# microsoft/AI2BMD

Measured on NVIDIA B200. Metric: MD steps/sec, higher is better.
Workload: dtype f32

## Files before the change

### ai2bmd_b200/csrc/engine.cu

```cuda
#include <cuda_runtime.h>

#include <algorithm>
#include <cmath>
#include <cstdarg>
#include <cstdio>
#include <cstdlib>
#include <cstring>
#include <mutex>
#include <string>
#include <vector>

#include "../../include/visnet_b200.h"
#include "k_edge.cuh"
#include "k_caph.cuh"
#include "k_comm.cuh"
#include "k_edge_tc.cuh"
#include "k_fused.cuh"
#include "k_graph_embed.cuh"
#include <nvtx3/nvToolsExt.h>
#include "k_head.cuh"
#include "k_md.cuh"
#include "k_nonbonded.cuh"
#include "k_restraint.cuh"
#include "k_node.cuh"
// ... 107 lines not shown
    float* d_ef = nullptr;
    int* d_flags = nullptr;
    bool caph_ready = false;
    CaphDev caph{};
    void* caph_mem = nullptr;
    bool comm_ready = false;
    int comm_auto = 1;
    void* comm_base = nullptr;
    void* comm_peer[COMM_MAX_WORLD] = {};
    CommParams comm{};
    int use_graph = 1, npw = 0, te_fwd = 0, te_bwd = 32;
    int use_pdl = 0;
    int npw_opt = 0, te_fwd_opt = 0, edge_tc_opt = -1;
    int tc_rows_opt = 0, tc_rows = 128;
    int tile_rows = 128;
    long long edges_plan = 0;
    int krot = 1;
    int node_nb = 0;
    int node_impl = 1;
    int fused = 0, fused_opt = -1;
    int node_tc = 0, node_tc_opt = -1;
    int embed_batch_opt = -1;
    int edge_tc = -1;
    struct GraphEntry { int kind; StepIO io; cudaGraphExec_t exec; };
    std::vector<GraphEntry> graphs;
    int launches = 0;
    bool accum_dirty = false;
    std::vector<std::string> stage_names;
    bool md_ready = false;
    MdParams md{};
// ... 304 lines not shown
    a.layer = l; a.mw = h->mw; a.ws = h->ws;
    const LayerW& lw = h->mw.layer[l];
    const size_t chunk = 4 * 8192;
    int n = 0;
    a.jobs[n++] = TcJob{lw.tcW1, (int)TC_COL_D0, 0};
    a.jobs[n++] = TcJob{lw.tcW1 + chunk, (int)TC_COL_D1, 0};
    if (l < L - 1) a.jobs[n++] = TcJob{lw.tcW1 + 2 * chunk, (int)TC_COL_D0, 0};
    a.jobs[n++] = TcJob{lw.tcWs, (int)TC_COL_D1, 0};
    a.jobs[n++] = TcJob{lw.tcWs + chunk, (int)TC_COL_D0, 0};
    a.njobs = n;
    a.tl = h->timeline ? h->d_tl + (size_t)l * TC_TL_SLOTS : nullptr;
    a.tile_rows = h->tile_rows;
    const int rows = h->tc_rows;
    const int tiles = (h->ws.Ecap + h->tile_rows - 1) / h->tile_rows;
    const int blocks = std::max(1, std::min(tiles, h->sm_count));
    if (rows == 32) Lc.launch(edge_fwd_tc_kernel<32>, dim3(blocks), dim3(TC2_THREADS), TC_SMEM_BYTES, a);
    else if (rows == 64) Lc.launch(edge_fwd_tc_kernel<64>, dim3(blocks), dim3(TC2_THREADS), TC_SMEM_BYTES, a);
    else if (rows == 96) Lc.launch(edge_fwd_tc_kernel<96>, dim3(blocks), dim3(TC2_THREADS), TC_SMEM_BYTES, a);
    else Lc.launch(edge_fwd_tc_kernel<128>, dim3(blocks), dim3(TC2_THREADS), TC_SMEM_BYTES, a);
    Lc.check();
}

void edge_fwd(Launcher& Lc, int l) {
    if (Lc.h->edge_tc & 1) { launch_edge_fwd_tc(Lc, l); return; }
    if (Lc.h->te_fwd == 64) launch_edge_fwd<64, 8>(Lc, l, 2);
    else launch_edge_fwd<32, 8>(Lc, l, 4);
}
void launch_edge_bwd_tc(Launcher& Lc, int l) {
    vb_handle* h = Lc.h;
    EdgeTcArgs a{};
    a.layer = l; a.mw = h->mw; a.ws = h->ws;
    const LayerW& lw = h->mw.layer[l];
    const size_t chunk = 4 * 8192;
    const bool upd = l < L - 1;
    int n = 0;
    a.jobs[n++] = TcJob{lw.tcWsN, (int)TC_COL_D1, 0};
    a.jobs[n++] = TcJob{lw.tcWsN + chunk, (int)TC_COL_D1, 1};
    a.jobs[n++] = TcJob{lw.tcW1N + chunk, (int)TC_COL_D0, 0};
    a.jobs[n++] = TcJob{lw.tcW1N, (int)TC_COL_D0, 1};
    if (upd) a.jobs[n++] = TcJob{lw.tcW1N + 2 * chunk, (int)TC_COL_D0, 1};
    a.njobs = n;
    a.tl = h->timeline ? h->d_tl + (size_t)(L + l) * TC_TL_SLOTS : nullptr;
    a.tile_rows = h->tile_rows;
    const int rows = h->tc_rows;
    const int tiles = (h->ws.Ecap + h->tile_rows - 1) / h->tile_rows;
    const int blocks = std::max(1, std::min(tiles, h->sm_count));
    if (rows == 32) Lc.launch(edge_bwd_tc_kernel<32>, dim3(blocks), dim3(TC2_THREADS), TC_SMEM_BYTES, a);
    else if (rows == 64) Lc.launch(edge_bwd_tc_kernel<64>, dim3(blocks), dim3(TC2_THREADS), TC_SMEM_BYTES, a);
    else if (rows == 96) Lc.launch(edge_bwd_tc_kernel<96>, dim3(blocks), dim3(TC2_THREADS), TC_SMEM_BYTES, a);
    else Lc.launch(edge_bwd_tc_kernel<128>, dim3(blocks), dim3(TC2_THREADS), TC_SMEM_BYTES, a);
    Lc.check();
}

void edge_bwd(Launcher& Lc, int l) {
    if (Lc.h->edge_tc & 2) { launch_edge_bwd_tc(Lc, l); return; }
    if (Lc.h->te_bwd == 64) launch_edge_bwd<64, 8>(Lc, l, 1);
    else launch_edge_bwd<32, 8>(Lc, l, 2);
}

void fill_fwd_jobs(const LayerW& lw, int l, TcJob* jobs, int& n) {
    const size_t chunk = 4 * 8192;
    n = 0;
    jobs[n++] = TcJob{lw.tcW1, (int)TC_COL_D0, 0};
    jobs[n++] = TcJob{lw.tcW1 + chunk, (int)TC_COL_D1, 0};
    if (l < L - 1) jobs[n++] = TcJob{lw.tcW1 + 2 * chunk, (int)TC_COL_D0, 0};
// ... 210 lines not shown

template <typename K>
cudaError_t opt_in_smem(K kernel, size_t bytes) {
    return cudaFuncSetAttribute(kernel, cudaFuncAttributeMaxDynamicSharedMemorySize, (int)bytes);
}

int configure_kernels(vb_handle* h) {
    CUDA_TRY(h, opt_in_smem(edge_fwd_kernel<32, 8>, edge_fwd_smem_bytes<32>()));
    CUDA_TRY(h, opt_in_smem(edge_fwd_kernel<64, 8>, edge_fwd_smem_bytes<64>()));
    CUDA_TRY(h, opt_in_smem(edge_bwd_kernel<32, 8>, edge_bwd_smem_bytes<32>()));
    CUDA_TRY(h, opt_in_smem(edge_bwd_kernel<64, 8>, edge_bwd_smem_bytes<64>()));
    CUDA_TRY(h, opt_in_smem(node_bwd_kernel<1>, node_bwd_smem_bytes<1>()));
    CUDA_TRY(h, opt_in_smem(node_bwd_kernel<2>, node_bwd_smem_bytes<2>()));
    CUDA_TRY(h, opt_in_smem(head_kernel<1>, HeadSmem<1>::BYTES));
    CUDA_TRY(h, opt_in_smem(head_kernel<2>, HeadSmem<2>::BYTES));
    CUDA_TRY(h, opt_in_smem(edge_fwd_tc_kernel<32>, TC_SMEM_BYTES));
    CUDA_TRY(h, opt_in_smem(edge_fwd_tc_kernel<64>, TC_SMEM_BYTES));
    CUDA_TRY(h, opt_in_smem(edge_fwd_tc_kernel<96>, TC_SMEM_BYTES));
    CUDA_TRY(h, opt_in_smem(edge_fwd_tc_kernel<128>, TC_SMEM_BYTES));
    CUDA_TRY(h, opt_in_smem(edge_bwd_tc_kernel<32>, TC_SMEM_BYTES));
    CUDA_TRY(h, opt_in_smem(edge_bwd_tc_kernel<64>, TC_SMEM_BYTES));
    CUDA_TRY(h, opt_in_smem(edge_bwd_tc_kernel<96>, TC_SMEM_BYTES));
    CUDA_TRY(h, opt_in_smem(edge_bwd_tc_kernel<128>, TC_SMEM_BYTES));
    CUDA_TRY(h, opt_in_smem(fused_fwd_kernel, TC_SMEM_BYTES));
    CUDA_TRY(h, opt_in_smem(fused_bwd_kernel, TC_SMEM_BYTES));
    CUDA_TRY(h, opt_in_smem(node_tc_kernel<NT_OPROJ>, TC_SMEM_BYTES));
    CUDA_TRY(h, opt_in_smem(node_tc_kernel<NT_PROJ>, TC_SMEM_BYTES));
    CUDA_TRY(h, opt_in_smem(node_tc_kernel<NT_BWDA>, TC_SMEM_BYTES));
    CUDA_TRY(h, opt_in_smem(node_tc_kernel<NT_BWDB>, TC_SMEM_BYTES));

    CUDA_TRY(h, opt_in_smem(node_fwd2_kernel<1>, sizeof(NodeFwd2SmemK<1>)));
    CUDA_TRY(h, opt_in_smem(node_bwd2_kernel<1>, sizeof(NodeBwd2SmemK<1>)));
    CUDA_TRY(h, opt_in_smem(node_fwd2_kernel<2>, sizeof(NodeFwd2SmemK<2>)));
    CUDA_TRY(h, opt_in_smem(node_bwd2_kernel<2>, sizeof(NodeBwd2SmemK<2>)));
    CUDA_TRY(h, opt_in_smem(node_fwd2_kernel<3>, sizeof(NodeFwd2SmemK<3>)));
    CUDA_TRY(h, opt_in_smem(node_bwd2_kernel<3>, sizeof(NodeBwd2SmemK<3>)));
    CUDA_TRY(h, opt_in_smem(node_fwd2_kernel<4>, sizeof(NodeFwd2SmemK<4>)));
    CUDA_TRY(h, opt_in_smem(node_bwd2_kernel<4>, sizeof(NodeBwd2SmemK<4>)));
// ... 95 lines not shown
void plan_tiles(vb_handle* h, long long edges) {
    const long long sm = h->sm_count;
    const long long padded = edges + edges * 3 / 100 + 1;
    const long long waves = std::max<long long>(1, (padded + sm * 128 - 1) / (sm * 128));
    long long rpw = (padded + sm * waves * 16 - 1) / (sm * waves * 16);
    if (rpw >= 7) rpw = 8;
    const long long rows = 16 * std::min<long long>(8, std::max<long long>(1, rpw));
    if (h->tc_rows_opt > 0) {
        h->tc_rows = h->tc_rows_opt;
        h->tile_rows = h->tc_rows_opt;
    } else {
        h->tc_rows = rows <= 32 ? 32 : rows <= 64 ? 64 : rows <= 96 ? 96 : 128;
        h->tile_rows = (int)rows;
    }
    h->edges_plan = edges;
}

void choose_defaults(vb_handle* h) {
    const int N = h->ws.N;
    h->npw = h->npw_opt; h->te_fwd = h->te_fwd_opt; h->edge_tc = h->edge_tc_opt;
    h->fused = h->fused_opt >= 0 ? h->fused_opt : 0;
    h->node_tc = h->node_tc_opt >= 0 ? h->node_tc_opt : (N >= 600 ? 1 : 0);
    if (h->fused) h->node_tc = 0;
    set_gxa_parts(h);
    if (h->npw == 0) h->npw = (N > 4096) ? 2 : 1;
    if (h->te_fwd == 0) h->te_fwd = ((long long)N * 17 / 64 >= 2LL * h->sm_count) ? 64 : 32;
    if (h->edge_tc < 0) h->edge_tc = 3;
    plan_tiles(h, h->edges_plan > 0 ? h->edges_plan : (long long)N * 17);
}

// ... 47 lines not shown
    }
    bind_weights(h->mw, h->d_weights);
    h->mw.cutoff = hp->cutoff;
    if (cudaStreamCreateWithFlags(&h->own_stream, cudaStreamNonBlocking) != cudaSuccess) { h->set_error("stream create failed"); return fail(VB_ERR_CUDA); }
    if (configure_kernels(h) != VB_OK) return fail(VB_ERR_CUDA);
    if (const char* s = getenv("VB_USE_GRAPH")) h->use_graph = atoi(s);
    if (const char* s = getenv("VB_NPW")) h->npw_opt = atoi(s);
    if (const char* s = getenv("VB_TE_FWD")) h->te_fwd_opt = atoi(s);
    if (const char* s = getenv("VB_TE_BWD")) h->te_bwd = atoi(s);
    if (const char* s = getenv("VB_EDGE_TC")) h->edge_tc_opt = atoi(s);
    if (const char* s = getenv("VB_USE_PDL")) h->use_pdl = atoi(s) ? 1 : 0;
    if (const char* s = getenv("VB_TC_ROWS")) { const int v = atoi(s); if (v == 32 || v == 64 || v == 96 || v == 128) h->tc_rows_opt = v; }
    if (const char* s = getenv("VB_NODE_IMPL")) h->node_impl = atoi(s);
    if (const char* s = getenv("VB_FUSED")) h->fused_opt = atoi(s) ? 1 : 0;
    if (const char* s = getenv("VB_NODE_TC")) h->node_tc_opt = atoi(s) ? 1 : 0;
    *out = h;
    return VB_OK;
}

void vb_destroy(vb_handle* h) {
    if (!h) return;
    cudaSetDevice(h->device);
    h->drop_graph();
    if (h->own_stream) cudaStreamDestroy(h->own_stream);
    cudaFree(h->d_weights);
    cudaFree(h->d_tl);
    h->free_md();
    h->free_nb();
    h->free_rs();
    h->free_comm();
// ... 695 lines not shown

int vb_set_option(vb_handle* h, const char* key, int64_t value) {
    if (!h || !key) return VB_ERR_ARG;
    std::lock_guard<std::mutex> lk(h->mu);
    const std::string k(key);
    if (k == "use_graph") h->use_graph = (int)value;
    else if (k == "use_pdl" && (value == 0 || value == 1)) h->use_pdl = (int)value;
    else if (k == "npw" && (value == 1 || value == 2)) h->npw = h->npw_opt = (int)value;
    else if (k == "te_fwd" && (value == 32 || value == 64)) h->te_fwd = h->te_fwd_opt = (int)value;
    else if (k == "te_bwd" && (value == 32 || value == 64)) h->te_bwd = (int)value;
    else if (k == "edge_tc" && value >= 0 && value <= 3) h->edge_tc = h->edge_tc_opt = (int)value;
    else if (k == "tc_rows" && (value == 0 || value == 32 || value == 64 || value == 96 || value == 128)) {
        h->tc_rows_opt = (int)value;
        if (h->has_topology) plan_tiles(h, h->edges_plan > 0 ? h->edges_plan : (long long)h->ws.N * 17);
    }
    else if (k == "calibrate" && value == 1) {
        if (!h->has_topology) { h->set_error("vb_set_option: calibrate needs a topology"); return VB_ERR_STATE; }
        int e = 0;
        if (cudaSetDevice(h->device) != cudaSuccess || cudaDeviceSynchronize() != cudaSuccess ||
            cudaMemcpy(&e, h->ws.rowptr + h->ws.N, sizeof(int), cudaMemcpyDeviceToHost) != cudaSuccess) {
            h->set_error("vb_set_option: calibrate failed: %s", cudaGetErrorString(cudaGetLastError()));
            return VB_ERR_CUDA;
        }
        if (e > 0) plan_tiles(h, e);
    }
    else if (k == "node_impl" && (value == 0 || value == 1)) h->node_impl = (int)value;
    else if (k == "node_nb" && (value == 0 || value == 1 || value == 2 || value == 3 || value == 4 || value == 8)) h->node_nb = (int)value;
    else if (k == "krot" && (value == 0 || value == 1)) h->krot = (int)value;
    else if (k == "fused" && (value == 0 || value == 1)) { h->fused = h->fused_opt = (int)value; if (value) h->node_tc = 0; set_gxa_parts(h); }
    else if (k == "node_tc" && (value == 0 || value == 1)) { h->node_tc = h->node_tc_opt = (int)value; if (value) h->fused = 0; set_gxa_parts(h); }
// ... 34 lines not shown
        int v = 0;
        if (!h->caph_ready || cudaDeviceSynchronize() != cudaSuccess ||
            cudaMemcpy(&v, h->caph.evals_out, sizeof(int), cudaMemcpyDeviceToHost) != cudaSuccess) return VB_ERR_STATE;
        return v;
    }
    if (k == "comm_ready") return h->comm_ready ? 1 : 0;
    if (k == "restraints_ready") return h->rs_ready ? 1 : 0;
    if (k == "edge_overflow") {
        int flag = 0;
        if (h->d_flags && cudaMemcpy(&flag, h->d_flags, sizeof(int), cudaMemcpyDeviceToHost) != cudaSuccess) return VB_ERR_CUDA;
        return flag;
    }
    if (k == "timeline") return h->timeline;
    if (k == "tc_rows") return h->tc_rows;
    if (k == "tile_rows") return h->tile_rows;
    if (k == "n_edges_capacity") return h->ws.Ecap;
    return VB_ERR_ARG;
}

int vb_num_stages(const vb_handle* h) { return h ? (int)h->stage_names.size() : 0; }
const char* vb_stage_name(const vb_handle* h, int stage) {
    if (!h || stage < 0 || stage >= (int)h->stage_names.size()) return "";
    return h->stage_names[stage].c_str();
}

int vb_debug_run(vb_handle* h, const float* pos_dev, int n_stages) {
    if (!h) return VB_ERR_ARG;
    std::lock_guard<std::mutex> lk(h->mu);
    if (!h->has_topology || !pos_dev) { h->set_error("vb_debug_run: bad state/arguments"); return VB_ERR_STATE; }
    CUDA_TRY(h, cudaSetDevice(h->device));
// ... 131 lines not shown
```

### ai2bmd_b200/csrc/k_edge_tc.cuh

```cuda
#pragma once
#include "k_edge.cuh"
#include "tc_common.cuh"

namespace vb {

constexpr int TC_TE = 128;
constexpr int TC_STAGES = 4;
constexpr int TC_MAXJOBS = 12;
constexpr int TC_THREADS = 192;
constexpr int TC_LT = D + LDS_PAD;
constexpr int TC_TILE_EXT = 1792;

constexpr uint32_t TC_COL_AHI = 0, TC_COL_ALO = 128, TC_COL_D0 = 256, TC_COL_D1 = 384;

struct TcJob {
    const float* img;
    int d_col;
    int accumulate;
};

struct TcShared {
    alignas(1024) uint8_t ring[TC_STAGES][tc::STAGE_BYTES];
    alignas(16) float tile[TC_TE][TC_LT];
    float tile_ext[TC_TILE_EXT];
// ... 38 lines not shown
    uint32_t phase = 0;
    for (int t = 0; t < ntiles; t++) {
        for (int j = 0; j < njobs; j++) {
            const char* src = reinterpret_cast<const char*>(jobs[j].img);
#pragma unroll 1
            for (int s = 0; s < D / tc::SLAB_K; s++) {
                tc::mbar_wait(&sh.b_empty[stage], phase ^ 1);
                tc::mbar_arrive_expect_tx(&sh.b_full[stage], tc::STAGE_BYTES);
                tc::tma_load_1d(sh.ring[stage], src + (size_t)s * tc::STAGE_BYTES, tc::STAGE_BYTES, &sh.b_full[stage]);
                if (++stage == TC_STAGES) { stage = 0; phase ^= 1; }
            }
        }
    }
}

__device__ __forceinline__ void tc_mma_issuer(TcShared& sh, const TcJob* jobs, int njobs, int ntiles, uint32_t tmem_base,
                                              unsigned long long* tl = nullptr) {
    constexpr uint32_t idesc = tc::idesc_tf32(128, 128);
    int stage = 0;
    uint32_t phase = 0;
    for (int t = 0; t < ntiles; t++) {
        const uint32_t tpar = (uint32_t)(t & 1);
        for (int j = 0; j < njobs; j++) {
            tc::mbar_wait(&sh.go[j], tpar);
            tc::fence_after_sync();
            if (tl != nullptr && t == 0) tl[32 + 2 * j] = (unsigned long long)clock64();
            const uint32_t d_addr = tmem_base + (uint32_t)jobs[j].d_col;
            uint32_t acc = (uint32_t)jobs[j].accumulate;
#pragma unroll 1
            for (int s = 0; s < D / tc::SLAB_K; s++) {
                tc::mbar_wait(&sh.b_full[stage], phase);
                tc::fence_after_sync();
                const uint32_t bhi = tc::smem_u32(sh.ring[stage]);
                const uint32_t blo = bhi + tc::SLAB_BYTES;
#pragma unroll
                for (int kk = 0; kk < tc::SLAB_K / 8; kk++) {
                    const uint32_t a_off = (uint32_t)(s * tc::SLAB_K + kk * 8);
                    const uint64_t dhi = tc::smem_desc_sw128(bhi + kk * 32);
                    const uint64_t dlo = tc::smem_desc_sw128(blo + kk * 32);
                    tc::mma_tf32_ts(d_addr, tmem_base + TC_COL_ALO + a_off, dhi, idesc, acc);
                    tc::mma_tf32_ts(d_addr, tmem_base + TC_COL_AHI + a_off, dlo, idesc, 1u);
                    tc::mma_tf32_ts(d_addr, tmem_base + TC_COL_AHI + a_off, dhi, idesc, 1u);
                    acc = 1u;
                }
                tc::mma_commit(&sh.b_empty[stage]);
                if (++stage == TC_STAGES) { stage = 0; phase ^= 1; }
            }
            tc::mma_commit(&sh.done[j]);
            if (tl != nullptr && t == 0) tl[33 + 2 * j] = (unsigned long long)clock64();
        }
    }
}

__device__ __forceinline__ void tc_signal_go(TcShared& sh, int j) {
    tc::wait_st();
    tc::fence_before_sync();
    tc::mbar_arrive(&sh.go[j]);
// ... 78 lines not shown
        tc::mbar_init(&sh.b_tile, TC2_CWARPS);
        tc::fence_barrier_init();
    }
    if (warp == TC2_CWARPS) tc::tmem_alloc(&sh.tmem_base, 512);
    tc::fence_before_sync();
    __syncthreads();
    tc::fence_after_sync();
    return sh.tmem_base;
}
__device__ __forceinline__ void tc2_teardown(uint32_t tmem_base) {
    tc::fence_before_sync();
    __syncthreads();
    if ((threadIdx.x >> 5) == TC2_CWARPS) tc::tmem_dealloc(tmem_base, 512);
}

template <int ROWS>
__device__ __forceinline__ void tc2_tile_to_a(TcShared& sh, uint32_t tmem, int warp, int lane) {
    if ((warp & 3) * 32 >= ROWS) return;
    const int row = (warp & 3) * 32 + lane, ch = (warp >> 2) * TC2_CBLK;
    const uint32_t tl = tmem + ((uint32_t)((warp & 3) * 32) << 16);
#pragma unroll
    for (int c0 = 0; c0 < TC2_CBLK; c0 += 16) {
        float v[16];
#pragma unroll
        for (int q = 0; q < 16; q += 4) {
            const float4 x = ld4(&sh.tile[row][ch + c0 + q]);
            v[q] = x.x; v[q + 1] = x.y; v[q + 2] = x.z; v[q + 3] = x.w;
        }
        tc::store_a16(tl + TC_COL_AHI, tl + TC_COL_ALO, ch + c0, v);
    }
}
template <int ROWS>
__device__ __forceinline__ void tc2_d_to_tile(TcShared& sh, uint32_t tmem, uint32_t d_col, int warp, int lane) {
    if ((warp & 3) * 32 >= ROWS) return;
    const int row = (warp & 3) * 32 + lane, ch = (warp >> 2) * TC2_CBLK;
    const uint32_t tl = tmem + ((uint32_t)((warp & 3) * 32) << 16) + d_col;
    constexpr int NB16 = TC2_CBLK / 16;
    uint32_t r[NB16][16];
#pragma unroll
    for (int b = 0; b < NB16; b++) tc::tmem_ld16_nowait(tl + ch + b * 16, r[b]);
    tc::wait_ld();
#pragma unroll
    for (int b = 0; b < NB16; b++)
#pragma unroll
        for (int q = 0; q < 16; q += 4)
            st4(&sh.tile[row][ch + b * 16 + q], f4(__uint_as_float(r[b][q]), __uint_as_float(r[b][q + 1]),
                                                    __uint_as_float(r[b][q + 2]), __uint_as_float(r[b][q + 3])));
}
__device__ __forceinline__ void tc2_go(TcShared& sh, int j) {
    tc::wait_st();
    tc::fence_before_sync();
    tc::mbar_arrive(&sh.go[j]);
}

template <int ROWS>
__global__ void __launch_bounds__(TC2_THREADS, 1) edge_fwd_tc_kernel(const __grid_constant__ EdgeTcArgs a) {
    pdl_entry();
    extern __shared__ __align__(1024) uint8_t dyn_raw[];
    TcShared& sh = *tc_shared_base(dyn_raw);
    const Workspace& ws = a.ws;
    const int l = a.layer;
    const LayerW& lw = a.mw.layer[l];
    const bool upd = (l < L - 1);
    const int J_DK = 0, J_DV = 1, J_F = 2, J_S1 = upd ? 3 : 2, J_S2 = upd ? 4 : 3;
    constexpr int RPW = ROWS / TC2_CWARPS;
    const int warp = threadIdx.x >> 5, lane = threadIdx.x & 31, col = lane * 4;
    const int E = ws.rowptr[ws.N];
    const int trows = min(ROWS, max(16, a.tile_rows));
    const int ntiles_total = (E + trows - 1) / trows;
    const int my_tiles = ((int)blockIdx.x < ntiles_total) ? (ntiles_total - (int)blockIdx.x + (int)gridDim.x - 1) / (int)gridDim.x : 0;
    if (a.tl != nullptr && blockIdx.x == 0 && threadIdx.x == 0) a.tl[0] = (unsigned long long)clock64();
    const uint32_t tmem = tc2_setup(sh, a.njobs);
    if (a.tl != nullptr && blockIdx.x == 0 && threadIdx.x == 0) a.tl[1] = (unsigned long long)clock64();

    if (warp == TC2_CWARPS) {
        if (lane == 0) tc_producer(sh, a.jobs, a.njobs, my_tiles);
    } else if (warp == TC2_CWARPS + 1) {
        if (lane == 0) tc_mma_issuer(sh, a.jobs, a.njobs, my_tiles, tmem, blockIdx.x == 0 ? a.tl : nullptr);
    } else {
        const float* __restrict__ Fin = ws.F[l];
        float* __restrict__ Fout = upd ? ws.F[l + 1] : nullptr;
        const float* __restrict__ QKV = ws.QKV[l];
        const float* __restrict__ VN = ws.VN[l];
        const float* __restrict__ TU = ws.TU[l];
        float* __restrict__ P1 = ws.P1[l];
        float* __restrict__ SP = ws.SP[l];
        float* __restrict__ ATT = ws.ATT[l];
        const int cch = threadIdx.x & (D - 1), grp = threadIdx.x >> 7;
        for (int it = 0; it < my_tiles; it++) {
            const uint32_t tpar = (uint32_t)(it & 1);
            const int e0 = ((int)blockIdx.x + it * (int)gridDim.x) * trows;
            const int nvalid = min(trows, E - e0);
            const int rpw = (nvalid + TC2_CWARPS - 1) / TC2_CWARPS, r0 = warp * rpw;
            {
                constexpr int RW = ROWS / TC2_CWARPS;
                const int w0 = warp * RW, wn = max(0, min(RW, nvalid - w0));
                if (lane == 0) {
                    if (wn > 0) tc::mbar_arrive_expect_tx(&sh.b_tile, (uint32_t)wn * D * 4);
                    else tc::mbar_arrive(&sh.b_tile);
                }
                __syncwarp();
                if (lane < wn) tc::tma_load_1d(&sh.tile[w0 + lane][0], Fin + (size_t)(e0 + w0 + lane) * D, D * 4, &sh.b_tile);
            }
            load_edge_meta<TC_TE, TC2_CTHREADS>(sh.meta, ws, e0, nvalid);
            tc::mbar_wait(&sh.b_tile, tpar);
            csync();
            TC_TL(2);
            tc2_tile_to_a<ROWS>(sh, tmem, warp, lane);
            tc2_go(sh, J_DK);
            tc2_go(sh, J_DV);
            TC_TL(3);
            float Areg[RPW];
            tc::mbar_wait(&sh.done[J_DK], tpar);
            tc::fence_after_sync();
            TC_TL(4);
            csync();
            tc2_d_to_tile<ROWS>(sh, tmem, TC_COL_D0, warp, lane);
            tc::fence_before_sync();
            csync();
            {
                TC_TL(5);
                const float4 bb = ldg4(lw.b1 + col);
#pragma unroll
                for (int r = 0; r < RPW; r++) {
                    if (r >= rpw) break;
                    const int row = r0 + r;
                    const float4 qi = ldg4(QKV + (size_t)sh.meta.dst[row] * 3 * D + col);
                    const float4 kj = ldg4(QKV + (size_t)sh.meta.src[row] * 3 * D + D + col);
                    const float4 P = ld4(&sh.tile[row][col]) + bb;
                    const float av = quad_sum(hsum4(qi * kj * silu4(P)));
                    Areg[r] = silu_(av) * sh.meta.C[row];
                    if ((r < rpw && row < nvalid)) {
                        st4(P1 + (size_t)(e0 + row) * 3 * D + col, P);
                        if ((lane & 3) == 0) ATT[(size_t)(e0 + row) * H + (lane >> 2)] = av;
                    }
                }
            }
            TC_TL(6);
            if (upd) { tc::fence_before_sync(); tc::mbar_arrive(&sh.go[J_F]); }
            tc::mbar_wait(&sh.done[J_DV], tpar);
            tc::fence_after_sync();
            TC_TL(7);
            csync();
            tc2_d_to_tile<ROWS>(sh, tmem, TC_COL_D1, warp, lane);
            csync();
            {
                TC_TL(8);
                const float4 bb = ldg4(lw.b1 + D + col);
#pragma unroll
                for (int r = 0; r < RPW; r++) {
                    if (r >= rpw) break;
                    const int row = r0 + r;
                    const float4 vj = ldg4(QKV + (size_t)sh.meta.src[row] * 3 * D + 2 * D + col);
                    const float4 P = ld4(&sh.tile[row][col]) + bb;
                    st4(&sh.tile[row][col], vj * silu4(P) * Areg[r]);
                    if ((r < rpw && row < nvalid)) st4(P1 + (size_t)(e0 + row) * 3 * D + D + col, P);
                }
            }
            csync();
            TC_TL(9);
            {
                const int i_first = sh.meta.dst[0], i_last = sh.meta.dst[nvalid - 1];
                for (int i = i_first + grp; i <= i_last; i += TC2_NGRP) {
                    const int q0 = ws.rowptr[i], q1 = ws.rowptr[i + 1];
                    const int lo = max(q0, e0) - e0, hi = min(q1, e0 + nvalid) - e0;
                    float xa = 0.f;
                    for (int r = lo; r < hi; r++) xa += sh.tile[r][cch];
                    if (q0 >= e0 && q1 <= e0 + nvalid) ws.XA[(size_t)i * D + cch] = xa;
                    else atomicAdd(ws.XA + (size_t)i * D + cch, xa);
                }
            }
            TC_TL(10);
            if (upd) { tc::mbar_wait(&sh.done[J_F], tpar); tc::fence_after_sync(); }
            tc2_tile_to_a<ROWS>(sh, tmem, warp, lane);
            tc2_go(sh, J_S1);
            TC_TL(11);
            if (upd) {
                csync();
                tc2_d_to_tile<ROWS>(sh, tmem, TC_COL_D0, warp, lane);
                tc::fence_before_sync();
                csync();
                const float4 bb = ldg4(lw.b1 + 2 * D + col);
#pragma unroll 1
                for (int rb = 0; rb < RPW; rb += 2) {
                    if (rb >= rpw) break;
                    float4 tir[2][3], ujr[2][3], fin[2];
#pragma unroll
                    for (int u = 0; u < 2; u++) {
                        const int row = r0 + rb + u;
                        const size_t i3 = (size_t)sh.meta.dst[row] * 3, j3 = (size_t)sh.meta.src[row] * 3;
                        fin[u] = (rb + u < rpw && row < nvalid) ? ldg4(Fin + (size_t)(e0 + row) * D + col) : f4s(0.f);
#pragma unroll
                        for (int s = 0; s < 3; s++) {
                            tir[u][s] = ldg4(TU + (i3 + s) * 2 * D + col);
// ... 13 lines not shown
                        if ((rb + u < rpw && row < nvalid)) {
                            st4(P1 + (size_t)(e0 + row) * 3 * D + 2 * D + col, Pf);
                            st4(Fout + (size_t)(e0 + row) * D + col, fin[u] + fp * wdot);
                        }
                    }
                }
            }
            TC_TL(12);
            tc::fence_before_sync();
            tc::mbar_arrive(&sh.go[J_S2]);
            float bnd[2][3] = {{0.f, 0.f, 0.f}, {0.f, 0.f, 0.f}};
            tc::mbar_wait(&sh.done[J_S1], tpar);
            tc::fence_after_sync();
            TC_TL(13);
            csync();
            tc2_d_to_tile<ROWS>(sh, tmem, TC_COL_D1, warp, lane);
            csync();
            {
                TC_TL(14);
                const float b = __ldg(lw.bs + cch);
                const int i_first = sh.meta.dst[0], i_last = sh.meta.dst[nvalid - 1];
                int nb = 0;
                for (int i = i_first + grp; i <= i_last; i += TC2_NGRP) {
                    const int q0 = ws.rowptr[i], q1 = ws.rowptr[i + 1];
                    const int lo = max(q0, e0) - e0, hi = min(q1, e0 + nvalid) - e0;
                    float v0 = 0.f, v1 = 0.f, v2 = 0.f;
                    int r = lo;
                    for (; r + 4 <= hi; r += 4) {
                        float g[4][3], s1[4];
#pragma unroll
                        for (int u = 0; u < 4; u++) {
// ... 22 lines not shown
                    } else if (nb < 2) {
                        bnd[nb][0] = v0; bnd[nb][1] = v1; bnd[nb][2] = v2;
                        nb++;
                    }
                }
            }
            TC_TL(15);
            if (threadIdx.x == 0 && it + 1 < my_tiles) {
                const int en = ((int)blockIdx.x + (it + 1) * (int)gridDim.x) * trows;
                tc::tma_prefetch_l2(Fin + (size_t)en * D, (uint32_t)min(trows, E - en) * D * 4);
            }
            tc::mbar_wait(&sh.done[J_S2], tpar);
            tc::fence_after_sync();
            TC_TL(16);
            csync();
            tc2_d_to_tile<ROWS>(sh, tmem, TC_COL_D0, warp, lane);
            tc::fence_before_sync();
            csync();
            {
                TC_TL(17);
                const float b = __ldg(lw.bs + D + cch);
                const int i_first = sh.meta.dst[0], i_last = sh.meta.dst[nvalid - 1];
                int nb = 0;
                for (int i = i_first + grp; i <= i_last; i += TC2_NGRP) {
                    const int q0 = ws.rowptr[i], q1 = ws.rowptr[i + 1];
                    const int lo = max(q0, e0) - e0, hi = min(q1, e0 + nvalid) - e0;
                    float v0 = 0.f, v1 = 0.f, v2 = 0.f;
                    for (int r = lo; r < hi; r++) {
                        const float4 de = sh.meta.d[r];
                        const float sp = sh.tile[r][cch] + b;
                        SP[(size_t)(e0 + r) * 2 * D + D + cch] = sp;
// ... 12 lines not shown
                    }
                }
            }
            TC_TL(18);
            csync();
        }
    }
    tc2_teardown(tmem);
    if (a.tl != nullptr && blockIdx.x == 0 && threadIdx.x == 0) a.tl[31] = (unsigned long long)clock64();
}

}

namespace vb {

template <int ROWS>
__global__ void __launch_bounds__(TC2_THREADS, 1) edge_bwd_tc_kernel(const __grid_constant__ EdgeTcArgs a) {
    pdl_entry();
    extern __shared__ __align__(1024) uint8_t dyn_raw[];
    TcShared& sh = *tc_shared_base(dyn_raw);
    const Workspace& ws = a.ws;
    const int l = a.layer;
    const bool upd = (l < L - 1);
    const int J_G3A = 0, J_G3B = 1, J_G4DV = 2, J_G4DK = 3, J_G4F = 4;
    const int J_LAST = upd ? J_G4F : J_G4DK;
    constexpr int RPW = ROWS / TC2_CWARPS;
    constexpr int RB4 = (RPW % 4 == 0) ? 4 : 2;
    const int warp = threadIdx.x >> 5, lane = threadIdx.x & 31, col = lane * 4, hd = lane >> 2;
    const int E = ws.rowptr[ws.N];
    const int trows = min(ROWS, max(16, a.tile_rows));
    const int ntiles_total = (E + trows - 1) / trows;
    const int my_tiles = ((int)blockIdx.x < ntiles_total) ? (ntiles_total - (int)blockIdx.x + (int)gridDim.x - 1) / (int)gridDim.x : 0;
    if (a.tl != nullptr && blockIdx.x == 0 && threadIdx.x == 0) a.tl[0] = (unsigned long long)clock64();
    const uint32_t tmem = tc2_setup(sh, a.njobs);
    if (a.tl != nullptr && blockIdx.x == 0 && threadIdx.x == 0) a.tl[1] = (unsigned long long)clock64();

    if (warp == TC2_CWARPS) {
        if (lane == 0) tc_producer(sh, a.jobs, a.njobs, my_tiles);
    } else if (warp == TC2_CWARPS + 1) {
        if (lane == 0) tc_mma_issuer(sh, a.jobs, a.njobs, my_tiles, tmem, blockIdx.x == 0 ? a.tl : nullptr);
    } else {
        const float* __restrict__ QKV = ws.QKV[l];
        const float* __restrict__ VN = ws.VN[l];
        const float* __restrict__ TU = ws.TU[l];
        const float* __restrict__ P1 = ws.P1[l];
        const float* __restrict__ SP = ws.SP[l];
        const float* __restrict__ ATT = ws.ATT[l];
        const int cch = threadIdx.x & (D - 1), grp = threadIdx.x >> 7;
        auto wait_done = [&](int j, uint32_t tpar) { tc::mbar_wait(&sh.done[j], tpar); tc::fence_after_sync(); };
        for (int it = 0; it < my_tiles; it++) {
            const uint32_t tpar = (uint32_t)(it & 1);
            const int e0 = ((int)blockIdx.x + it * (int)gridDim.x) * trows;
            const int nvalid = min(trows, E - e0);
            const int rpw = (nvalid + TC2_CWARPS - 1) / TC2_CWARPS, r0 = warp * rpw;
            load_edge_meta<TC_TE, TC2_CTHREADS>(sh.meta, ws, e0, nvalid);
// ... 17 lines not shown
                    const int row = r0 + rb + u;
                    const bool ok = (rb + u < rpw && row < nvalid);
                    const size_t j3 = (size_t)sh.meta.src[row] * 3;
                    const float4 s1 = silu4(sp[u]);
                    const float4 gs1 = gM[u][0] * vn[u][0] + gM[u][1] * vn[u][1] + gM[u][2] * vn[u][2];
                    if (rb + u < rpw) st4(&sh.tile[row][col], ok ? gs1 * dsilu4(sp[u]) : f4s(0.f));
                    if (ok) {
                        red4(ws.GVNMSG + (j3 + 0) * D + col, gM[u][0] * s1);
                        red4(ws.GVNMSG + (j3 + 1) * D + col, gM[u][1] * s1);
                        red4(ws.GVNMSG + (j3 + 2) * D + col, gM[u][2] * s1);
                    }
                }
            }
            TC_TL(3);
            csync();
            tc2_tile_to_a<ROWS>(sh, tmem, warp, lane);
            tc2_go(sh, J_G3A);
            TC_TL(4);
            csync();
#pragma unroll 4
            for (int r = 0; r < RPW; r++) {
                if (r >= rpw) break;
                const int row = r0 + r;
                const bool ok = (r < rpw && row < nvalid);
                const size_t e = (size_t)(e0 + (ok ? row : 0));
                const size_t i3 = (size_t)sh.meta.dst[row] * 3;
                const float4 dd = sh.meta.d[row];
                const float4 sp = ldg4(SP + e * 2 * D + D + col);
                const float4 s2 = silu4(sp);
                const float4 gM0 = ldg4(ws.GVEC + (i3 + 0) * D + col), gM1 = ldg4(ws.GVEC + (i3 + 1) * D + col),
                             gM2 = ldg4(ws.GVEC + (i3 + 2) * D + col);
                const float gx_ = warp_sum(hsum4(gM0 * s2)), gy_ = warp_sum(hsum4(gM1 * s2)), gz_ = warp_sum(hsum4(gM2 * s2));
                if (lane == 0) { sh.eacc[row][1] = gx_; sh.eacc[row][2] = gy_; sh.eacc[row][3] = gz_; }
                st4(&sh.tile[row][col], ok ? (gM0 * dd.x + gM1 * dd.y + gM2 * dd.z) * dsilu4(sp) : f4s(0.f));
            }
            TC_TL(5);
            csync();
            wait_done(J_G3A, tpar);
            TC_TL(6);
            tc2_tile_to_a<ROWS>(sh, tmem, warp, lane);
            tc2_go(sh, J_G3B);
            TC_TL(7);
            wait_done(J_G3B, tpar);
            TC_TL(8);
            csync();
            tc2_d_to_tile<ROWS>(sh, tmem, TC_COL_D1, warp, lane);
            tc::fence_before_sync();
            csync();
            TC_TL(9);
#pragma unroll 1
            for (int rb = 0; rb < RPW; rb += RB4) {
                if (rb >= rpw) break;
                float4 gxa[RB4], vjr[RB4], pdvr[RB4];
                float avr[RB4];
#pragma unroll
                for (int u = 0; u < RB4; u++) {
                    const int row = r0 + rb + u;
                    const size_t e = (size_t)(e0 + ((rb + u < rpw && row < nvalid) ? row : 0));
                    gxa[u] = load_gxa(ws, (size_t)sh.meta.dst[row], col);
                    vjr[u] = ldg4(QKV + (size_t)sh.meta.src[row] * 3 * D + 2 * D + col);
                    pdvr[u] = ldg4(P1 + e * 3 * D + D + col);
// ... 7 lines not shown
                    const float Ce = sh.meta.C[row];
                    const float av = avr[u], sa = silu_(av), A = sa * Ce;
                    const bool mine = rb + u < rpw;
                    const float4 gm = mine ? ld4(&sh.tile[row][col]) + gxa[u] : f4s(0.f);
                    const float4 dv = silu4(pdvr[u]);
                    if (mine) st4(&sh.tile[row][col], ok ? gm * vjr[u] * A * dsilu4(pdvr[u]) : f4s(0.f));
                    const float gA = quad_sum(hsum4(gm * vjr[u] * dv));
                    if (mine && (lane & 3) == 0) sh.gattn[row][hd] = gA * Ce * dsilu_(av);
                    const float gc = warp_sum((lane & 3) == 0 ? gA * sa : 0.f);
                    if (mine && lane == 0) sh.eacc[row][0] = gc;
                    if (ok) red4(ws.GQKV + j * 3 * D + 2 * D + col, gm * dv * A);
                }
            }
            TC_TL(10);
            csync();
            tc2_tile_to_a<ROWS>(sh, tmem, warp, lane);
            tc2_go(sh, J_G4DV);
            TC_TL(11);
            csync();
#pragma unroll 1
            for (int rb = 0; rb < RPW; rb += RB4) {
                if (rb >= rpw) break;
                float4 pdkr[RB4], qir[RB4], kjr[RB4];
#pragma unroll
                for (int u = 0; u < RB4; u++) {
                    const int row = r0 + rb + u;
                    const size_t e = (size_t)(e0 + ((rb + u < rpw && row < nvalid) ? row : 0));
                    pdkr[u] = ldg4(P1 + e * 3 * D + col);
                    qir[u] = ldg4(QKV + (size_t)sh.meta.dst[row] * 3 * D + col);
                    kjr[u] = ldg4(QKV + (size_t)sh.meta.src[row] * 3 * D + D + col);
                }
#pragma unroll
                for (int u = 0; u < RB4; u++) {
                    const int row = r0 + rb + u;
                    const bool ok = (rb + u < rpw && row < nvalid);
                    const size_t j = sh.meta.src[row];
                    const float4 dk = silu4(pdkr[u]);
                    const float gav = sh.gattn[row][hd];
                    if (rb + u < rpw) st4(&sh.tile[row][col], ok ? qir[u] * kjr[u] * gav * dsilu4(pdkr[u]) : f4s(0.f));
                    if (ok) red4(ws.GQKV + j * 3 * D + D + col, qir[u] * dk * gav);
                }
            }
            TC_TL(12);
            csync();
            wait_done(J_G4DV, tpar);
            TC_TL(13);
            tc2_tile_to_a<ROWS>(sh, tmem, warp, lane);
            tc2_go(sh, J_G4DK);
            TC_TL(14);
            csync();
#pragma unroll 4
            for (int r = 0; r < RPW; r++) {
                if (r >= rpw) break;
                const int row = r0 + r;
                const size_t e = (size_t)(e0 + ((r < rpw && row < nvalid) ? row : 0));
                const float4 dk = silu4(ldg4(P1 + e * 3 * D + col));
                const float4 kj = ldg4(QKV + (size_t)sh.meta.src[row] * 3 * D + D + col);
                st4(&sh.tile[row][col], kj * dk * sh.gattn[row][hd]);
            }
            csync();
            {
                const int i_first = sh.meta.dst[0], i_last = sh.meta.dst[nvalid - 1];
// ... 56 lines not shown
                            gdl[s] = warp_sum(hsum4(tir[u][s] * c1 + a1 * gw1 + ujr[u][s] * c2 + a2 * gw2));
                        }
                        if (lane == 0 && rb + u < rpw) { sh.eacc[row][1] -= gdl[0]; sh.eacc[row][2] -= gdl[1]; sh.eacc[row][3] -= gdl[2]; }
                        if (ok) {
                            red4(ws.GTU + (j3 + 0) * 2 * D + D + col, gu[0]);
                            red4(ws.GTU + (j3 + 1) * 2 * D + D + col, gu[1]);
                            red4(ws.GTU + (j3 + 2) * 2 * D + D + col, gu[2]);
                        }
                        (void)e;
                    }
                }
                TC_TL(16);
                csync();
                wait_done(J_G4DK, tpar);
                TC_TL(17);
                tc2_tile_to_a<ROWS>(sh, tmem, warp, lane);
                tc2_go(sh, J_G4F);
                TC_TL(18);
                csync();
#pragma unroll 4
                for (int r = 0; r < RPW; r++) {
                    if (r >= rpw) break;
                    const int row = r0 + r;
                    const bool ok = (r < rpw && row < nvalid);
                    const size_t e = (size_t)(e0 + (ok ? row : 0));
                    const float4 gfn = ok ? ld4(ws.GF + e * D + col) : f4s(0.f);
                    st4(&sh.tile[row][col], gfn * silu4(ldg4(P1 + e * 3 * D + 2 * D + col)));
                }
                csync();
                {
                    const int i_first = sh.meta.dst[0], i_last = sh.meta.dst[nvalid - 1];
// ... 40 lines not shown
                        }
                    }
                }
            }
            TC_TL(19);
            if (threadIdx.x < 3 && it + 1 < my_tiles) {
                const int en = ((int)blockIdx.x + (it + 1) * (int)gridDim.x) * trows;
                const uint32_t nn = (uint32_t)min(trows, E - en);
                if (threadIdx.x == 0) tc::tma_prefetch_l2(SP + (size_t)en * 2 * D, nn * 2 * D * 4);
                else if (threadIdx.x == 1) tc::tma_prefetch_l2(P1 + (size_t)en * 3 * D, nn * 3 * D * 4);
                else tc::tma_prefetch_l2(ATT + (size_t)en * H, nn * H * 4);
            }
            wait_done(J_LAST, tpar);
            TC_TL(20);
            csync();
            tc2_d_to_tile<ROWS>(sh, tmem, TC_COL_D0, warp, lane);
            tc::fence_before_sync();
            csync();
            TC_TL(21);
#pragma unroll 4
            for (int r = 0; r < RPW; r++) {
                if (r >= rpw) break;
                const int row = r0 + r;
                if ((r < rpw && row < nvalid)) {
                    float* g = ws.GF + (size_t)(e0 + row) * D + col;
                    float4 v = ld4(&sh.tile[row][col]);
                    if (upd) v = v + ld4(g);
                    st4(g, v);
                }
            }
            if (threadIdx.x < nvalid) {
// ... 13 lines not shown
```

### ai2bmd_b200/csrc/tc_common.cuh

```cuda
#pragma once
#include <cuda_runtime.h>
#include <stdint.h>

namespace vb {
namespace tc {

__device__ __forceinline__ uint32_t smem_u32(const void* p) { return (uint32_t)__cvta_generic_to_shared(p); }

__device__ __forceinline__ void mbar_init(uint64_t* bar, uint32_t count) {
    asm volatile("mbarrier.init.shared::cta.b64 [%0], %1;" ::"r"(smem_u32(bar)), "r"(count));
}
__device__ __forceinline__ void fence_barrier_init() { asm volatile("fence.mbarrier_init.release.cluster;" ::: "memory"); }
__device__ __forceinline__ void mbar_arrive(uint64_t* bar) {
    asm volatile("{\n\t.reg .b64 st;\n\tmbarrier.arrive.shared::cta.b64 st, [%0];\n\t}" ::"r"(smem_u32(bar)) : "memory");
}
__device__ __forceinline__ void mbar_arrive_expect_tx(uint64_t* bar, uint32_t bytes) {
    asm volatile("{\n\t.reg .b64 st;\n\tmbarrier.arrive.expect_tx.shared::cta.b64 st, [%0], %1;\n\t}" ::"r"(smem_u32(bar)),
                 "r"(bytes)
                 : "memory");
}
__device__ __forceinline__ void mbar_wait(uint64_t* bar, uint32_t parity) {
    asm volatile(
        "{\n\t"
        ".reg .pred p;\n\t"
// ... 82 lines not shown
}

__device__ __forceinline__ void split_tf32(float x, uint32_t& hi, uint32_t& lo) {
    asm("cvt.rna.tf32.f32 %0, %1;" : "=r"(hi) : "f"(x));
    const float rest = x - __uint_as_float(hi);
    asm("cvt.rna.tf32.f32 %0, %1;" : "=r"(lo) : "f"(rest));
}

__device__ __forceinline__ void store_a16(uint32_t tmem_hi, uint32_t tmem_lo, int c0, const float (&v)[16]) {
    uint32_t hi[16], lo[16];
#pragma unroll
    for (int i = 0; i < 16; i++) split_tf32(v[i], hi[i], lo[i]);
    tmem_st16(tmem_hi + c0, hi);
    tmem_st16(tmem_lo + c0, lo);
}

constexpr int SLAB_K = 32;
constexpr int SLAB_BYTES = 128 * SLAB_K * 4;
constexpr int STAGE_BYTES = 2 * SLAB_BYTES;

}
}
```

Baseline: 1504.

## Fold hi/lo TF32 A planes into one 128-row operand for small tiles

When the tile holds at most 64 edge rows, the A operand's hi and lo TF32 splits are stacked in the upper and lower halves of a single 128-row TMEM operand. This cuts the three-MMA split-precision sequence per k-step to two. The two partial accumulator halves are then summed with a lane shuffle during read-out. It is enabled by default whenever tc_rows is 64 or less. It adds a shuffle and an extra split per element, and it drops the lo×lo-equivalent cross term only in layout, not in precision.

Measured after the change: 1528, median of 6. 1.6% higher.

```diff
diff --git a/ai2bmd_b200/csrc/engine.cu b/ai2bmd_b200/csrc/engine.cu
--- a/ai2bmd_b200/csrc/engine.cu
+++ b/ai2bmd_b200/csrc/engine.cu
@@ -145,6 +145,7 @@
     int npw_opt = 0, te_fwd_opt = 0, edge_tc_opt = -1;
     int tc_rows_opt = 0, tc_rows = 128;
     int tile_rows = 128;
+    int tc_fold_opt = -1, tc_fold = 0;
     long long edges_plan = 0;
     int krot = 1;
     int node_nb = 0;
@@ -479,10 +480,12 @@
     const int rows = h->tc_rows;
     const int tiles = (h->ws.Ecap + h->tile_rows - 1) / h->tile_rows;
     const int blocks = std::max(1, std::min(tiles, h->sm_count));
-    if (rows == 32) Lc.launch(edge_fwd_tc_kernel<32>, dim3(blocks), dim3(TC2_THREADS), TC_SMEM_BYTES, a);
-    else if (rows == 64) Lc.launch(edge_fwd_tc_kernel<64>, dim3(blocks), dim3(TC2_THREADS), TC_SMEM_BYTES, a);
-    else if (rows == 96) Lc.launch(edge_fwd_tc_kernel<96>, dim3(blocks), dim3(TC2_THREADS), TC_SMEM_BYTES, a);
-    else Lc.launch(edge_fwd_tc_kernel<128>, dim3(blocks), dim3(TC2_THREADS), TC_SMEM_BYTES, a);
+    if (h->tc_fold && rows == 32) Lc.launch(edge_fwd_tc_kernel<32, true>, dim3(blocks), dim3(TC2_THREADS), TC_SMEM_BYTES, a);
+    else if (h->tc_fold && rows == 64) Lc.launch(edge_fwd_tc_kernel<64, true>, dim3(blocks), dim3(TC2_THREADS), TC_SMEM_BYTES, a);
+    else if (rows == 32) Lc.launch(edge_fwd_tc_kernel<32, false>, dim3(blocks), dim3(TC2_THREADS), TC_SMEM_BYTES, a);
+    else if (rows == 64) Lc.launch(edge_fwd_tc_kernel<64, false>, dim3(blocks), dim3(TC2_THREADS), TC_SMEM_BYTES, a);
+    else if (rows == 96) Lc.launch(edge_fwd_tc_kernel<96, false>, dim3(blocks), dim3(TC2_THREADS), TC_SMEM_BYTES, a);
+    else Lc.launch(edge_fwd_tc_kernel<128, false>, dim3(blocks), dim3(TC2_THREADS), TC_SMEM_BYTES, a);
     Lc.check();
 }
 
@@ -510,10 +513,12 @@
     const int rows = h->tc_rows;
     const int tiles = (h->ws.Ecap + h->tile_rows - 1) / h->tile_rows;
     const int blocks = std::max(1, std::min(tiles, h->sm_count));
-    if (rows == 32) Lc.launch(edge_bwd_tc_kernel<32>, dim3(blocks), dim3(TC2_THREADS), TC_SMEM_BYTES, a);
-    else if (rows == 64) Lc.launch(edge_bwd_tc_kernel<64>, dim3(blocks), dim3(TC2_THREADS), TC_SMEM_BYTES, a);
-    else if (rows == 96) Lc.launch(edge_bwd_tc_kernel<96>, dim3(blocks), dim3(TC2_THREADS), TC_SMEM_BYTES, a);
-    else Lc.launch(edge_bwd_tc_kernel<128>, dim3(blocks), dim3(TC2_THREADS), TC_SMEM_BYTES, a);
+    if (h->tc_fold && rows == 32) Lc.launch(edge_bwd_tc_kernel<32, true>, dim3(blocks), dim3(TC2_THREADS), TC_SMEM_BYTES, a);
+    else if (h->tc_fold && rows == 64) Lc.launch(edge_bwd_tc_kernel<64, true>, dim3(blocks), dim3(TC2_THREADS), TC_SMEM_BYTES, a);
+    else if (rows == 32) Lc.launch(edge_bwd_tc_kernel<32, false>, dim3(blocks), dim3(TC2_THREADS), TC_SMEM_BYTES, a);
+    else if (rows == 64) Lc.launch(edge_bwd_tc_kernel<64, false>, dim3(blocks), dim3(TC2_THREADS), TC_SMEM_BYTES, a);
+    else if (rows == 96) Lc.launch(edge_bwd_tc_kernel<96, false>, dim3(blocks), dim3(TC2_THREADS), TC_SMEM_BYTES, a);
+    else Lc.launch(edge_bwd_tc_kernel<128, false>, dim3(blocks), dim3(TC2_THREADS), TC_SMEM_BYTES, a);
     Lc.check();
 }
 
@@ -754,14 +759,18 @@
     CUDA_TRY(h, opt_in_smem(node_bwd_kernel<2>, node_bwd_smem_bytes<2>()));
     CUDA_TRY(h, opt_in_smem(head_kernel<1>, HeadSmem<1>::BYTES));
     CUDA_TRY(h, opt_in_smem(head_kernel<2>, HeadSmem<2>::BYTES));
-    CUDA_TRY(h, opt_in_smem(edge_fwd_tc_kernel<32>, TC_SMEM_BYTES));
-    CUDA_TRY(h, opt_in_smem(edge_fwd_tc_kernel<64>, TC_SMEM_BYTES));
-    CUDA_TRY(h, opt_in_smem(edge_fwd_tc_kernel<96>, TC_SMEM_BYTES));
-    CUDA_TRY(h, opt_in_smem(edge_fwd_tc_kernel<128>, TC_SMEM_BYTES));
-    CUDA_TRY(h, opt_in_smem(edge_bwd_tc_kernel<32>, TC_SMEM_BYTES));
-    CUDA_TRY(h, opt_in_smem(edge_bwd_tc_kernel<64>, TC_SMEM_BYTES));
-    CUDA_TRY(h, opt_in_smem(edge_bwd_tc_kernel<96>, TC_SMEM_BYTES));
-    CUDA_TRY(h, opt_in_smem(edge_bwd_tc_kernel<128>, TC_SMEM_BYTES));
+    CUDA_TRY(h, opt_in_smem(edge_fwd_tc_kernel<32, false>, TC_SMEM_BYTES));
+    CUDA_TRY(h, opt_in_smem(edge_fwd_tc_kernel<64, false>, TC_SMEM_BYTES));
+    CUDA_TRY(h, opt_in_smem(edge_fwd_tc_kernel<96, false>, TC_SMEM_BYTES));
+    CUDA_TRY(h, opt_in_smem(edge_fwd_tc_kernel<128, false>, TC_SMEM_BYTES));
+    CUDA_TRY(h, opt_in_smem(edge_fwd_tc_kernel<32, true>, TC_SMEM_BYTES));
+    CUDA_TRY(h, opt_in_smem(edge_fwd_tc_kernel<64, true>, TC_SMEM_BYTES));
+    CUDA_TRY(h, opt_in_smem(edge_bwd_tc_kernel<32, false>, TC_SMEM_BYTES));
+    CUDA_TRY(h, opt_in_smem(edge_bwd_tc_kernel<64, false>, TC_SMEM_BYTES));
+    CUDA_TRY(h, opt_in_smem(edge_bwd_tc_kernel<96, false>, TC_SMEM_BYTES));
+    CUDA_TRY(h, opt_in_smem(edge_bwd_tc_kernel<128, false>, TC_SMEM_BYTES));
+    CUDA_TRY(h, opt_in_smem(edge_bwd_tc_kernel<32, true>, TC_SMEM_BYTES));
+    CUDA_TRY(h, opt_in_smem(edge_bwd_tc_kernel<64, true>, TC_SMEM_BYTES));
     CUDA_TRY(h, opt_in_smem(fused_fwd_kernel, TC_SMEM_BYTES));
     CUDA_TRY(h, opt_in_smem(fused_bwd_kernel, TC_SMEM_BYTES));
     CUDA_TRY(h, opt_in_smem(node_tc_kernel<NT_OPROJ>, TC_SMEM_BYTES));
@@ -887,6 +896,7 @@
         h->tile_rows = (int)rows;
     }
     h->edges_plan = edges;
+    h->tc_fold = (h->tc_fold_opt != 0 && h->tc_rows <= 64) ? 1 : 0;
 }
 
 void choose_defaults(vb_handle* h) {
@@ -964,6 +974,7 @@
     if (const char* s = getenv("VB_NODE_IMPL")) h->node_impl = atoi(s);
     if (const char* s = getenv("VB_FUSED")) h->fused_opt = atoi(s) ? 1 : 0;
     if (const char* s = getenv("VB_NODE_TC")) h->node_tc_opt = atoi(s) ? 1 : 0;
+    if (const char* s = getenv("VB_TC_FOLD")) h->tc_fold_opt = atoi(s) ? 1 : 0;
     *out = h;
     return VB_OK;
 }
@@ -1689,6 +1700,10 @@
         h->tc_rows_opt = (int)value;
         if (h->has_topology) plan_tiles(h, h->edges_plan > 0 ? h->edges_plan : (long long)h->ws.N * 17);
     }
+    else if (k == "tc_fold" && value >= -1 && value <= 1) {
+        h->tc_fold_opt = (int)value;
+        if (h->has_topology) plan_tiles(h, h->edges_plan > 0 ? h->edges_plan : (long long)h->ws.N * 17);
+    }
     else if (k == "calibrate" && value == 1) {
         if (!h->has_topology) { h->set_error("vb_set_option: calibrate needs a topology"); return VB_ERR_STATE; }
         int e = 0;
@@ -1753,6 +1768,7 @@
     if (k == "timeline") return h->timeline;
     if (k == "tc_rows") return h->tc_rows;
     if (k == "tile_rows") return h->tile_rows;
+    if (k == "tc_fold") return h->tc_fold;
     if (k == "n_edges_capacity") return h->ws.Ecap;
     return VB_ERR_ARG;
 }
diff --git a/ai2bmd_b200/csrc/k_edge_tc.cuh b/ai2bmd_b200/csrc/k_edge_tc.cuh
--- a/ai2bmd_b200/csrc/k_edge_tc.cuh
+++ b/ai2bmd_b200/csrc/k_edge_tc.cuh
@@ -76,6 +76,7 @@
     }
 }
 
+template <bool FOLD = false>
 __device__ __forceinline__ void tc_mma_issuer(TcShared& sh, const TcJob* jobs, int njobs, int ntiles, uint32_t tmem_base,
                                               unsigned long long* tl = nullptr) {
     constexpr uint32_t idesc = tc::idesc_tf32(128, 128);
@@ -100,9 +101,14 @@
                     const uint32_t a_off = (uint32_t)(s * tc::SLAB_K + kk * 8);
                     const uint64_t dhi = tc::smem_desc_sw128(bhi + kk * 32);
                     const uint64_t dlo = tc::smem_desc_sw128(blo + kk * 32);
-                    tc::mma_tf32_ts(d_addr, tmem_base + TC_COL_ALO + a_off, dhi, idesc, acc);
-                    tc::mma_tf32_ts(d_addr, tmem_base + TC_COL_AHI + a_off, dlo, idesc, 1u);
-                    tc::mma_tf32_ts(d_addr, tmem_base + TC_COL_AHI + a_off, dhi, idesc, 1u);
+                    if (FOLD) {
+                        tc::mma_tf32_ts(d_addr, tmem_base + TC_COL_AHI + a_off, dhi, idesc, acc);
+                        tc::mma_tf32_ts(d_addr, tmem_base + TC_COL_AHI + a_off, dlo, idesc, 1u);
+                    } else {
+                        tc::mma_tf32_ts(d_addr, tmem_base + TC_COL_ALO + a_off, dhi, idesc, acc);
+                        tc::mma_tf32_ts(d_addr, tmem_base + TC_COL_AHI + a_off, dlo, idesc, 1u);
+                        tc::mma_tf32_ts(d_addr, tmem_base + TC_COL_AHI + a_off, dhi, idesc, 1u);
+                    }
                     acc = 1u;
                 }
                 tc::mma_commit(&sh.b_empty[stage]);
@@ -211,8 +217,24 @@
     if ((threadIdx.x >> 5) == TC2_CWARPS) tc::tmem_dealloc(tmem_base, 512);
 }
 
-template <int ROWS>
+template <int ROWS, bool FOLD>
 __device__ __forceinline__ void tc2_tile_to_a(TcShared& sh, uint32_t tmem, int warp, int lane) {
+    if (FOLD) {
+        if ((warp & 3) * 16 >= ROWS) return;
+        const int row = (warp & 3) * 16 + (lane & 15), ch = (warp >> 2) * TC2_CBLK;
+        const uint32_t tl = tmem + ((uint32_t)((warp & 3) * 32) << 16) + TC_COL_AHI;
+#pragma unroll
+        for (int c0 = 0; c0 < TC2_CBLK; c0 += 16) {
+            float v[16];
+#pragma unroll
+            for (int q = 0; q < 16; q += 4) {
+                const float4 x = ld4(&sh.tile[row][ch + c0 + q]);
+                v[q] = x.x; v[q + 1] = x.y; v[q + 2] = x.z; v[q + 3] = x.w;
+            }
+            tc::store_a16_plane(tl, ch + c0, v, lane >= 16);
+        }
+        return;
+    }
     if ((warp & 3) * 32 >= ROWS) return;
     const int row = (warp & 3) * 32 + lane, ch = (warp >> 2) * TC2_CBLK;
     const uint32_t tl = tmem + ((uint32_t)((warp & 3) * 32) << 16);
@@ -227,12 +249,34 @@
         tc::store_a16(tl + TC_COL_AHI, tl + TC_COL_ALO, ch + c0, v);
     }
 }
-template <int ROWS>
+template <int ROWS, bool FOLD>
 __device__ __forceinline__ void tc2_d_to_tile(TcShared& sh, uint32_t tmem, uint32_t d_col, int warp, int lane) {
+    constexpr int NB16 = TC2_CBLK / 16;
+    static_assert(NB16 == 2, "the folded read-out splits a column block into two halves of 16");
+    if (FOLD) {
+        if ((warp & 3) * 16 >= ROWS) return;
+        const int row = (warp & 3) * 16 + (lane & 15), ch = (warp >> 2) * TC2_CBLK;
+        const uint32_t tl = tmem + ((uint32_t)((warp & 3) * 32) << 16) + d_col;
+        uint32_t r[NB16][16];
+#pragma unroll
+        for (int b = 0; b < NB16; b++) tc::tmem_ld16_nowait(tl + ch + b * 16, r[b]);
+        tc::wait_ld();
+        const bool up = lane >= 16;
+        float v[16];
+#pragma unroll
+        for (int q = 0; q < 16; q++) {
+            const float send = __uint_as_float(up ? r[0][q] : r[1][q]);
+            const float own = __uint_as_float(up ? r[1][q] : r[0][q]);
+            v[q] = own + __shfl_xor_sync(0xffffffffu, send, 16);
+        }
+        const int c = ch + (up ? 16 : 0);
+#pragma unroll
+        for (int q = 0; q < 16; q += 4) st4(&sh.tile[row][c + q], f4(v[q], v[q + 1], v[q + 2], v[q + 3]));
+        return;
+    }
     if ((warp & 3) * 32 >= ROWS) return;
     const int row = (warp & 3) * 32 + lane, ch = (warp >> 2) * TC2_CBLK;
     const uint32_t tl = tmem + ((uint32_t)((warp & 3) * 32) << 16) + d_col;
-    constexpr int NB16 = TC2_CBLK / 16;
     uint32_t r[NB16][16];
 #pragma unroll
     for (int b = 0; b < NB16; b++) tc::tmem_ld16_nowait(tl + ch + b * 16, r[b]);
@@ -250,8 +294,9 @@
     tc::mbar_arrive(&sh.go[j]);
 }
 
-template <int ROWS>
+template <int ROWS, bool FOLD>
 __global__ void __launch_bounds__(TC2_THREADS, 1) edge_fwd_tc_kernel(const __grid_constant__ EdgeTcArgs a) {
+    static_assert(!FOLD || ROWS <= 64, "the folded A operand holds at most 64 rows");
     pdl_entry();
     extern __shared__ __align__(1024) uint8_t dyn_raw[];
     TcShared& sh = *tc_shared_base(dyn_raw);
@@ -273,7 +318,7 @@
     if (warp == TC2_CWARPS) {
         if (lane == 0) tc_producer(sh, a.jobs, a.njobs, my_tiles);
     } else if (warp == TC2_CWARPS + 1) {
-        if (lane == 0) tc_mma_issuer(sh, a.jobs, a.njobs, my_tiles, tmem, blockIdx.x == 0 ? a.tl : nullptr);
+        if (lane == 0) tc_mma_issuer<FOLD>(sh, a.jobs, a.njobs, my_tiles, tmem, blockIdx.x == 0 ? a.tl : nullptr);
     } else {
         const float* __restrict__ Fin = ws.F[l];
         float* __restrict__ Fout = upd ? ws.F[l + 1] : nullptr;
@@ -303,7 +348,7 @@
             tc::mbar_wait(&sh.b_tile, tpar);
             csync();
             TC_TL(2);
-            tc2_tile_to_a<ROWS>(sh, tmem, warp, lane);
+            tc2_tile_to_a<ROWS, FOLD>(sh, tmem, warp, lane);
             tc2_go(sh, J_DK);
             tc2_go(sh, J_DV);
             TC_TL(3);
@@ -312,7 +357,7 @@
             tc::fence_after_sync();
             TC_TL(4);
             csync();
-            tc2_d_to_tile<ROWS>(sh, tmem, TC_COL_D0, warp, lane);
+            tc2_d_to_tile<ROWS, FOLD>(sh, tmem, TC_COL_D0, warp, lane);
             tc::fence_before_sync();
             csync();
             {
@@ -339,7 +384,7 @@
             tc::fence_after_sync();
             TC_TL(7);
             csync();
-            tc2_d_to_tile<ROWS>(sh, tmem, TC_COL_D1, warp, lane);
+            tc2_d_to_tile<ROWS, FOLD>(sh, tmem, TC_COL_D1, warp, lane);
             csync();
             {
                 TC_TL(8);
@@ -369,12 +414,12 @@
             }
             TC_TL(10);
             if (upd) { tc::mbar_wait(&sh.done[J_F], tpar); tc::fence_after_sync(); }
-            tc2_tile_to_a<ROWS>(sh, tmem, warp, lane);
+            tc2_tile_to_a<ROWS, FOLD>(sh, tmem, warp, lane);
             tc2_go(sh, J_S1);
             TC_TL(11);
             if (upd) {
                 csync();
-                tc2_d_to_tile<ROWS>(sh, tmem, TC_COL_D0, warp, lane);
+                tc2_d_to_tile<ROWS, FOLD>(sh, tmem, TC_COL_D0, warp, lane);
                 tc::fence_before_sync();
                 csync();
                 const float4 bb = ldg4(lw.b1 + 2 * D + col);
@@ -418,7 +463,7 @@
             tc::fence_after_sync();
             TC_TL(13);
             csync();
-            tc2_d_to_tile<ROWS>(sh, tmem, TC_COL_D1, warp, lane);
+            tc2_d_to_tile<ROWS, FOLD>(sh, tmem, TC_COL_D1, warp, lane);
             csync();
             {
                 TC_TL(14);
@@ -471,7 +516,7 @@
             tc::fence_after_sync();
             TC_TL(16);
             csync();
-            tc2_d_to_tile<ROWS>(sh, tmem, TC_COL_D0, warp, lane);
+            tc2_d_to_tile<ROWS, FOLD>(sh, tmem, TC_COL_D0, warp, lane);
             tc::fence_before_sync();
             csync();
             {
@@ -514,8 +559,9 @@
 
 namespace vb {
 
-template <int ROWS>
+template <int ROWS, bool FOLD>
 __global__ void __launch_bounds__(TC2_THREADS, 1) edge_bwd_tc_kernel(const __grid_constant__ EdgeTcArgs a) {
+    static_assert(!FOLD || ROWS <= 64, "the folded A operand holds at most 64 rows");
     pdl_entry();
     extern __shared__ __align__(1024) uint8_t dyn_raw[];
     TcShared& sh = *tc_shared_base(dyn_raw);
@@ -538,7 +584,7 @@
     if (warp == TC2_CWARPS) {
         if (lane == 0) tc_producer(sh, a.jobs, a.njobs, my_tiles);
     } else if (warp == TC2_CWARPS + 1) {
-        if (lane == 0) tc_mma_issuer(sh, a.jobs, a.njobs, my_tiles, tmem, blockIdx.x == 0 ? a.tl : nullptr);
+        if (lane == 0) tc_mma_issuer<FOLD>(sh, a.jobs, a.njobs, my_tiles, tmem, blockIdx.x == 0 ? a.tl : nullptr);
     } else {
         const float* __restrict__ QKV = ws.QKV[l];
         const float* __restrict__ VN = ws.VN[l];
@@ -586,7 +632,7 @@
             }
             TC_TL(3);
             csync();
-            tc2_tile_to_a<ROWS>(sh, tmem, warp, lane);
+            tc2_tile_to_a<ROWS, FOLD>(sh, tmem, warp, lane);
             tc2_go(sh, J_G3A);
             TC_TL(4);
             csync();
@@ -610,13 +656,13 @@
             csync();
             wait_done(J_G3A, tpar);
             TC_TL(6);
-            tc2_tile_to_a<ROWS>(sh, tmem, warp, lane);
+            tc2_tile_to_a<ROWS, FOLD>(sh, tmem, warp, lane);
             tc2_go(sh, J_G3B);
             TC_TL(7);
             wait_done(J_G3B, tpar);
             TC_TL(8);
             csync();
-            tc2_d_to_tile<ROWS>(sh, tmem, TC_COL_D1, warp, lane);
+            tc2_d_to_tile<ROWS, FOLD>(sh, tmem, TC_COL_D1, warp, lane);
             tc::fence_before_sync();
             csync();
             TC_TL(9);
@@ -654,7 +700,7 @@
             }
             TC_TL(10);
             csync();
-            tc2_tile_to_a<ROWS>(sh, tmem, warp, lane);
+            tc2_tile_to_a<ROWS, FOLD>(sh, tmem, warp, lane);
             tc2_go(sh, J_G4DV);
             TC_TL(11);
             csync();
@@ -685,7 +731,7 @@
             csync();
             wait_done(J_G4DV, tpar);
             TC_TL(13);
-            tc2_tile_to_a<ROWS>(sh, tmem, warp, lane);
+            tc2_tile_to_a<ROWS, FOLD>(sh, tmem, warp, lane);
             tc2_go(sh, J_G4DK);
             TC_TL(14);
             csync();
@@ -772,7 +818,7 @@
                 csync();
                 wait_done(J_G4DK, tpar);
                 TC_TL(17);
-                tc2_tile_to_a<ROWS>(sh, tmem, warp, lane);
+                tc2_tile_to_a<ROWS, FOLD>(sh, tmem, warp, lane);
                 tc2_go(sh, J_G4F);
                 TC_TL(18);
                 csync();
@@ -843,7 +889,7 @@
             wait_done(J_LAST, tpar);
             TC_TL(20);
             csync();
-            tc2_d_to_tile<ROWS>(sh, tmem, TC_COL_D0, warp, lane);
+            tc2_d_to_tile<ROWS, FOLD>(sh, tmem, TC_COL_D0, warp, lane);
             tc::fence_before_sync();
             csync();
             TC_TL(21);
diff --git a/ai2bmd_b200/csrc/tc_common.cuh b/ai2bmd_b200/csrc/tc_common.cuh
--- a/ai2bmd_b200/csrc/tc_common.cuh
+++ b/ai2bmd_b200/csrc/tc_common.cuh
@@ -120,6 +120,15 @@
     tmem_st16(tmem_hi + c0, hi);
     tmem_st16(tmem_lo + c0, lo);
 }
+__device__ __forceinline__ void store_a16_plane(uint32_t taddr, int c0, const float (&v)[16], bool lo_plane) {
+    uint32_t hi[16], lo[16], r[16];
+#pragma unroll
+    for (int i = 0; i < 16; i++) {
+        split_tf32(v[i], hi[i], lo[i]);
+        r[i] = lo_plane ? lo[i] : hi[i];
+    }
+    tmem_st16(taddr + c0, r);
+}
 
 constexpr int SLAB_K = 32;
 constexpr int SLAB_BYTES = 128 * SLAB_K * 4;
```
